# zhaotudou/HeteroFusionRCNN

Measured on AMD Instinct MI355X. Metric: KITTI frames/sec RPN train step, higher is better.
Workload: dtype f32

## Files before the change

### heterofusionrcnn_amd/csrc/xconv.hip

```cpp
#include "xconv_common.h"

namespace hf {

template <int K, bool TRANSPOSED>
__global__ __launch_bounds__(kXcThreads) void xconv_apply_kernel(long long rows, int c, const float *__restrict__ x,
                                                                const float *__restrict__ f, float *__restrict__ out)
{
    const int lane = threadIdx.x & 63;
    const long long wave = __builtin_amdgcn_readfirstlane(static_cast<int>(threadIdx.x >> 6)) +
                           static_cast<long long>(blockIdx.x) * (kXcThreads / 64);
    const long long nwaves = static_cast<long long>(gridDim.x) * (kXcThreads / 64);
    for (long long r = wave; r < rows; r += nwaves) {
        const float *xr = x + r * (K * K);
        float coef[K][K];
#pragma unroll
        for (int i = 0; i < K; ++i)
#pragma unroll
            for (int j = 0; j < K; ++j) coef[i][j] = TRANSPOSED ? xr[j * K + i] : xr[i * K + j];
        const float *fr = f + r * K * c;
        float *orow = out + r * K * c;
        for (int ch = lane; ch < c; ch += 64) {
            float v[K];
#pragma unroll
            for (int j = 0; j < K; ++j) v[j] = fr[static_cast<size_t>(j) * c + ch];
// ... 296 lines not shown
                                                                    const float *__restrict__ grad_out, float *__restrict__ grad_f,
                                                                    float *__restrict__ grad_gathered, float *__restrict__ grad_wd,
                                                                    float *__restrict__ wd_partial)
{
    const int lane = threadIdx.x & 63, wave = __builtin_amdgcn_readfirstlane(static_cast<int>(threadIdx.x >> 6));
    const int ch = blockIdx.y * 64 + lane;
    const bool live = ch < c;
    const XcSource src = xc_source(live ? ch : blockIdx.y * 64, c, c0, f, fts, GATHER ? idx : nullptr);
    if (GATHER && src.gathered && !grad_wd && !grad_gathered) return;
    float w[K][M], gw[K][M];
#pragma unroll
    for (int k = 0; k < K; ++k)
#pragma unroll
        for (int m = 0; m < M; ++m) { w[k][m] = live ? wd[(static_cast<size_t>(k) * c + ch) * M + m] : 0.f; gw[k][m] = 0.f; }
    const long long r0 = static_cast<long long>(blockIdx.x) * rows_per_block;
    const long long r1 = r0 + rows_per_block < rows ? r0 + rows_per_block : rows;
    for (long long r = r0 + wave; r < r1; r += kXcThreads / 64) {
        const float *xr = x + r * (K * K);
        float fv[K], g[M], gfx[K];
        const long long tbase = (GATHER && src.gathered) ? static_cast<long long>(static_cast<unsigned>(r) / static_cast<unsigned>(rows_per_cloud)) * n_src : 0;
#pragma unroll
        for (int j = 0; j < K; ++j) {
            const long long srow = (GATHER && src.gathered) ? tbase + idx[r * K + j] : r * K + j;
            fv[j] = live ? src.base[srow * src.stride] : 0.f;
        }
        load_m<M>(grad_out, static_cast<size_t>(r * c + (live ? ch : 0)) * M, g);
        if (!live) {
#pragma unroll
            for (int m = 0; m < M; ++m) g[m] = 0.f;
        }
#pragma unroll
        for (int k = 0; k < K; ++k) {
            float a = 0.f;
#pragma unroll
            for (int m = 0; m < M; ++m) a = a + g[m] * w[k][m];
            gfx[k] = a;
            float t = xr[k * K] * fv[0];
#pragma unroll
            for (int j = 1; j < K; ++j) t = t + xr[k * K + j] * fv[j];
#pragma unroll
            for (int m = 0; m < M; ++m) gw[k][m] = gw[k][m] + t * g[m];
        }
        float *gdst = (GATHER && src.gathered) ? (grad_gathered ? grad_gathered + (ch - c0) : nullptr) : (grad_f ? grad_f + ch : nullptr);
        if (live && gdst) {
#pragma unroll
            for (int j = 0; j < K; ++j) {
                float a = xr[j] * gfx[0];
#pragma unroll
                for (int k = 1; k < K; ++k) a = a + xr[k * K + j] * gfx[k];
                gdst[(r * K + j) * src.stride] = a;
            }
        }
    }
    if (grad_wd) {
        __shared__ float red[K * M][64];
        for (int wv = 0; wv < kXcThreads / 64; ++wv) {
            if (wave == wv && live) {
#pragma unroll
                for (int k = 0; k < K; ++k)
#pragma unroll
                    for (int m = 0; m < M; ++m) red[k * M + m][lane] = wv == 0 ? gw[k][m] : red[k * M + m][lane] + gw[k][m];
            }
            __syncthreads();
        }
        float *mine = wd_partial ? wd_partial + static_cast<size_t>(blockIdx.x) * K * c * M : nullptr;
        for (int i = threadIdx.x; i < K * M * 64; i += kXcThreads) {
            const int km = i >> 6, c2 = blockIdx.y * 64 + (i & 63);
            if (c2 < c) {
                const size_t e = (static_cast<size_t>(km / M) * c + c2) * M + km % M;
                if (mine) mine[e] = red[km][i & 63];
                else atomicAdd(&grad_wd[e], red[km][i & 63]);
            }
        }
    }
}

template <int K, int M, bool GATHER>
__global__ __launch_bounds__(kXcThreads) void xconv_dw_bwd_x_kernel(long long rows, int c, int c0, const float *__restrict__ f,
                                                                   const float *__restrict__ fts, const int *__restrict__ idx, int n_src,
                                                                   int rows_per_cloud, const float *__restrict__ wd,
                                                                   const float *__restrict__ grad_out, float *__restrict__ grad_x)
{
    extern __shared__ float lds[];
    constexpr int KK = K * K, STRIDE = KK + 1, QUADS = 16;
    const int lane = threadIdx.x & 63, w = threadIdx.x >> 6;
    float *mine = lds + static_cast<size_t>(w) * QUADS * STRIDE;
    const long long wave = w + static_cast<long long>(blockIdx.x) * (kXcThreads / 64);
    const long long nwaves = static_cast<long long>(gridDim.x) * (kXcThreads / 64);
    const int c1 = c - c0;
    for (long long r = wave; r < rows; r += nwaves) {
        float acc[K][K];
#pragma unroll
        for (int i = 0; i < K; ++i)
#pragma unroll
            for (int j = 0; j < K; ++j) acc[i][j] = 0.f;
        long long trow[K];
        if constexpr (GATHER) {
            const long long tbase = static_cast<long long>(static_cast<unsigned>(r) / static_cast<unsigned>(rows_per_cloud)) * n_src;
#pragma unroll
            for (int j = 0; j < K; ++j) trow[j] = tbase + idx[r * K + j];
        }
        for (int ch = lane; ch < c; ch += 64) {
            float fv[K], g[M];
            if constexpr (GATHER) {
                const bool gathered = ch >= c0;
                const float *base = gathered ? fts + (ch - c0) : f + ch;
                const long long stride = gathered ? c1 : c0;
#pragma unroll
                for (int j = 0; j < K; ++j) fv[j] = base[(gathered ? trow[j] : r * K + j) * stride];
            } else {
#pragma unroll
                for (int j = 0; j < K; ++j) fv[j] = f[(r * K + j) * c + ch];
            }
            load_m<M>(grad_out, static_cast<size_t>(r * c + ch) * M, g);
#pragma unroll
            for (int k = 0; k < K; ++k) {
                float a = 0.f;
#pragma unroll
                for (int m = 0; m < M; ++m) a = a + g[m] * wd[(static_cast<size_t>(k) * c + ch) * M + m];
#pragma unroll
                for (int j = 0; j < K; ++j) acc[k][j] = acc[k][j] + a * fv[j];
            }
        }
#pragma unroll
        for (int i = 0; i < K; ++i)
#pragma unroll
            for (int j = 0; j < K; ++j) {
                float v = acc[i][j];
                v = v + __int_as_float(__builtin_amdgcn_mov_dpp(__float_as_int(v), 0xb1, 0xf, 0xf, true));
                v = v + __int_as_float(__builtin_amdgcn_mov_dpp(__float_as_int(v), 0x4e, 0xf, 0xf, true));
                if ((lane & 3) == 0) mine[(lane >> 2) * STRIDE + i * K + j] = v;
            }
        __builtin_amdgcn_fence(__ATOMIC_SEQ_CST, "wavefront");
        __builtin_amdgcn_wave_barrier();
        for (int p = lane; p < KK; p += 64) {
            float s = 0.f;
#pragma unroll
            for (int l = 0; l < QUADS; ++l) s = s + mine[l * STRIDE + p];
            grad_x[r * KK + p] = s;
        }
        __builtin_amdgcn_fence(__ATOMIC_SEQ_CST, "wavefront");
        __builtin_amdgcn_wave_barrier();
    }
}

constexpr int kFtsRows = 2, kFtsEntries = 4;
typedef float f4 __attribute__((ext_vector_type(4)));

constexpr int xc_fts_pairs(int m) { return m == 1 ? 2 : 1; }

template <int K, int M, bool VEC>
__global__ __launch_bounds__(kXcThreads) void xconv_dw_bwd_fts_kernel(long long src_rows, int n_src, long long rows_per_cloud,
                                                                     int c, int c0, int rows_per_block,
                                                                     const float *__restrict__ x, const float *__restrict__ wd,
                                                                     const float *grad_out,
                                                                     const int *__restrict__ offsets, const int *__restrict__ entries,
                                                                     float *grad_fts)
{
    constexpr int NP = xc_fts_pairs(M), CPL = 2 * NP, T = kFtsRows, E = kFtsEntries, NF = CPL * M, CHUNK = NF % 4 == 0 ? 4 : 2;
    constexpr int KP = K <= 4 ? 4 : (K <= 8 ? 8 : 16), QPL = 64 / KP, NR = (T * E + QPL - 1) / QPL;
    const int lane = threadIdx.x & 63, wave = __builtin_amdgcn_readfirstlane(static_cast<int>(threadIdx.x >> 6));
    const int lq = lane / KP, lk = lane % KP < K ? lane % KP : K - 1;
    const int c1 = c - c0, col0 = blockIdx.y * (64 * CPL), cf0 = col0 + lane * CPL;
    unsigned cc[CPL];
    bool live[CPL];
#pragma unroll
    for (int i = 0; i < CPL; ++i) {
        live[i] = cf0 + i < c1;
        cc[i] = static_cast<unsigned>(c0 + (live[i] ? cf0 + i : (VEC ? col0 + i : c1 - 1)));
    }
    f2 w[K][NP][M];
#pragma unroll
    for (int k = 0; k < K; ++k)
#pragma unroll
        for (int p = 0; p < NP; ++p)
#pragma unroll
            for (int m = 0; m < M; ++m)
                w[k][p][m] = f2{wd[(static_cast<size_t>(k) * c + cc[2 * p]) * M + m], wd[(static_cast<size_t>(k) * c + cc[2 * p + 1]) * M + m]};
    __shared__ __attribute__((aligned(16))) float xs[kXcThreads / 64][T * E][KP];
    const long long s0 = static_cast<long long>(blockIdx.x) * rows_per_block;
    const long long s1 = s0 + rows_per_block < src_rows ? s0 + rows_per_block : src_rows;
    long long bb = s0 / n_src;
    for (long long sb = s0 + wave * T; sb < s1; sb += (kXcThreads / 64) * T) {
        int pos[T], hi[T];
        long long ebase[T];
        unsigned rbase[T];
        f2 acc[T][NP];
        bool more = false;
#pragma unroll
        for (int t = 0; t < T; ++t) {
            const long long s = sb + t < s1 ? sb + t : s1 - 1;
            while (s >= (bb + 1) * n_src) ++bb;
            const int pt = static_cast<int>(s - bb * n_src);
            const int *off = offsets + bb * (n_src + 1);
            ebase[t] = bb * rows_per_cloud * K;
            rbase[t] = static_cast<unsigned>(bb * rows_per_cloud);
            pos[t] = off[pt];
            hi[t] = sb + t < s1 ? off[pt + 1] : pos[t];
            more = more || pos[t] < hi[t];
#pragma unroll
            for (int p = 0; p < NP; ++p) acc[t][p] = f2{0.f, 0.f};
        }
        auto load_slots = [&](int ahead, unsigned (&slot)[NR]) {
#pragma unroll
            for (int i = 0; i < NR; ++i) {
                const int q = i * QPL + lq < T * E ? i * QPL + lq : T * E - 1, u = q % E + ahead;
                int e = 0;
                long long eb = 0;
#pragma unroll
                for (int t = 0; t < T; ++t)
                    if (q / E == t) { e = pos[t] + u < hi[t] ? pos[t] + u : 0; eb = ebase[t]; }
                slot[i] = static_cast<unsigned>(entries[eb + e]);
            }
        };
        unsigned slot[NR], slot_next[NR];
        if (more) load_slots(0, slot);
        while (more) {
            unsigned rr[T * E];
            float xv[NR];
#pragma unroll
            for (int i = 0; i < NR; ++i) {
                const int q = i * QPL + lq < T * E ? i * QPL + lq : T * E - 1;
                unsigned rb = 0;
#pragma unroll
                for (int t = 0; t < T; ++t)
                    if (q / E == t) rb = rbase[t];
// ... 243 lines not shown
                                 as_stream(stream));
}

#define HF_XDW_DISPATCH(CALL)                                                                                          \
    if (k == 8 && m == 1) { CALL(8, 1) } else if (k == 8 && m == 2) { CALL(8, 2) } else if (k == 8 && m == 3) { CALL(8, 3) }      \
    else if (k == 8 && m == 4) { CALL(8, 4) }                                                                          \
    else if (k == 4 && m == 1) { CALL(4, 1) } else if (k == 4 && m == 4) { CALL(4, 4) }    \
    else if (k == 12 && m == 1) { CALL(12, 1) } else if (k == 12 && m == 2) { CALL(12, 2) }                             \
    else return HF_EINVAL;

static void xdw_grid(long long rows, int c, dim3 &grid, int &rows_per_block, int blocks_per_cu = 8, int chunk = 64)
{
    const int cchunks = div_up(c, chunk);
    long long rchunks = (blocks_per_cu * kNumCU + cchunks - 1) / cchunks;
    if (rchunks > (rows + 3) / 4) rchunks = (rows + 3) / 4;
    if (rchunks < 1) rchunks = 1;
    rows_per_block = static_cast<int>((rows + rchunks - 1) / rchunks);
    grid = dim3(static_cast<unsigned>((rows + rows_per_block - 1) / rows_per_block), cchunks);
}

bool hf::xdw_offsets_fit(long long rows, int k, int c, long long src_rows)
{
    return rows * k * static_cast<long long>(c) < (1ll << 32) && src_rows * static_cast<long long>(c) < (1ll << 32);
}

bool hf::xdw_v2(int c, std::initializer_list<const void *> ptrs)
{
    if (c & 1) return false;
    for (const void *p : ptrs)
        if (reinterpret_cast<uintptr_t>(p) & 7) return false;
    return true;
}

void hf::xdw_pair_grid(long long rows, int c, dim3 &grid, int &rpb, int blocks_per_cu) { xdw_grid(rows, c, grid, rpb, blocks_per_cu, 128); }

static int xdw_forward(long long rows, int k, int c, int c0, int m, const float *x, const float *f, const float *fts, const int *idx,
                       int n_src, int rows_per_cloud, const float *wd, float *out, hipStream_t st)
{
    if (!xdw_offsets_fit(rows, k, c, idx ? static_cast<long long>(rows / rows_per_cloud) * n_src : 0)) return HF_EINVAL;
    dim3 grid;
    int rpb;
    xdw_pair_grid(rows, c, grid, rpb, 8);
    const bool v2 = xdw_v2(c, {f, fts, out});
#define HF_XDW_FWD_V(KK, MM, V)                                                                                        \
    if (idx) hipLaunchKernelGGL((xconv_dw_fwd_kernel<KK, MM, true, V>), grid, dim3(kXcThreads), 0, st, rows, c, c0, rpb, x, f, fts, idx, n_src, rows_per_cloud, wd, out); \
    else hipLaunchKernelGGL((xconv_dw_fwd_kernel<KK, MM, false, V>), grid, dim3(kXcThreads), 0, st, rows, c, c0, rpb, x, f, fts, idx, n_src, rows_per_cloud, wd, out);
#define HF_XDW_FWD(KK, MM) if (v2) { HF_XDW_FWD_V(KK, MM, true) } else { HF_XDW_FWD_V(KK, MM, false) }
    HF_XDW_DISPATCH(HF_XDW_FWD)
#undef HF_XDW_FWD
#undef HF_XDW_FWD_V
    return launch_status();
}

void hf::xdw_bwd_grid(long long rows, int c, dim3 &grid, int &rpb)
{
    xdw_grid(rows, c, grid, rpb, 4);
    if (rpb < 32 && rows > 32) { rpb = 32; grid.x = static_cast<unsigned>((rows + rpb - 1) / rpb); }
}

static int xdw_backward(long long rows, int k, int c, int c0, int m, const float *x, const float *f, const float *fts, const int *idx,
                        int n_src, int rows_per_cloud, const float *wd, const float *grad_out, float *grad_x, float *grad_f, float *grad_gathered,
                        float *grad_wd, hipStream_t st, float *wd_partial = nullptr)
{
    if (grad_wd && (!wd_partial || rows == 0)) {
        const int rc = hip_status(hipMemsetAsync(grad_wd, 0, sizeof(float) * static_cast<size_t>(k) * c * m, st));
        if (rc != HF_OK) return rc;
    }
    if (rows == 0) return HF_OK;
    if (!grad_wd) wd_partial = nullptr;
    if (grad_f || grad_wd || grad_gathered) {
        dim3 grid;
        int rpb;
        xdw_bwd_grid(rows, c, grid, rpb);
#define HF_XDW_BFW(KK, MM)                                                                                             \
        if (idx) hipLaunchKernelGGL((xconv_dw_bwd_fw_kernel<KK, MM, true>), grid, dim3(kXcThreads), 0, st, rows, c, c0, rpb, x, f, fts, idx, n_src, rows_per_cloud, wd, grad_out, grad_f, grad_gathered, grad_wd, wd_partial); \
        else hipLaunchKernelGGL((xconv_dw_bwd_fw_kernel<KK, MM, false>), grid, dim3(kXcThreads), 0, st, rows, c, c0, rpb, x, f, fts, idx, n_src, rows_per_cloud, wd, grad_out, grad_f, grad_gathered, grad_wd, wd_partial);
        HF_XDW_DISPATCH(HF_XDW_BFW)
#undef HF_XDW_BFW
        if (wd_partial) launch_partial_reduce(k * c * m, static_cast<int>(grid.x), wd_partial, grad_wd, st);
        const int rc = launch_status();
        if (rc != HF_OK) return rc;
    }
    if (grad_x) {
        const size_t lds = sizeof(float) * (kXcThreads / 64) * 16 * (static_cast<size_t>(k) * k + 1);
#define HF_XDW_BX(KK, MM)                                                                                              \
        if (idx) hipLaunchKernelGGL((xconv_dw_bwd_x_kernel<KK, MM, true>), dim3(grid_for(rows, kXcThreads / 64)), dim3(kXcThreads), lds, st, rows, c, c0, f, fts, idx, n_src, rows_per_cloud, wd, grad_out, grad_x); \
        else hipLaunchKernelGGL((xconv_dw_bwd_x_kernel<KK, MM, false>), dim3(grid_for(rows, kXcThreads / 64)), dim3(kXcThreads), lds, st, rows, c, c0, f, fts, idx, n_src, rows_per_cloud, wd, grad_out, grad_x);
        HF_XDW_DISPATCH(HF_XDW_BX)
#undef HF_XDW_BX
        return launch_status();
    }
    return HF_OK;
}

HF_API int hf_xconv_depthwise(long long rows, int k, int c, int m, const float *x, const float *f, const float *wd, float *out,
                              hf_stream_t stream)
{
    if (rows < 0 || c <= 0 || !x || !f || !wd || !out) return HF_EINVAL;
    if (rows == 0) return HF_OK;
    return xdw_forward(rows, k, c, c, m, x, f, nullptr, nullptr, 0, 1, wd, out, as_stream(stream));
}

HF_API int hf_xconv_depthwise_grad(long long rows, int k, int c, int m, const float *x, const float *f, const float *wd,
                                   const float *grad_out, float *grad_x, float *grad_f, float *grad_wd, hf_stream_t stream)
{
    if (rows < 0 || c <= 0 || !x || !f || !wd || !grad_out || (!grad_x && !grad_f && !grad_wd)) return HF_EINVAL;
    return xdw_backward(rows, k, c, c, m, x, f, nullptr, nullptr, 0, 1, wd, grad_out, grad_x, grad_f, nullptr, grad_wd, as_stream(stream));
}

HF_API int hf_xconv_depthwise_gather(int b, int n_src, int rows_per_cloud, int k, int c0, int c1, int m, const float *x,
                                     const float *f_delta, const float *fts, const int *idx, const float *wd, float *out,
                                     hf_stream_t stream)
{
    if (b < 0 || n_src <= 0 || rows_per_cloud < 0 || c0 <= 0 || c0 % 64 != 0 || c1 <= 0) return HF_EINVAL;
    const long long rows = static_cast<long long>(b) * rows_per_cloud;
    if (rows == 0) return HF_OK;
    if (rows > 0x7fffffffll || !x || !f_delta || !fts || !idx || !wd || !out) return HF_EINVAL;
    return xdw_forward(rows, k, c0 + c1, c0, m, x, f_delta, fts, idx, n_src, rows_per_cloud, wd, out, as_stream(stream));
}

bool hf::xdw_fts_direct(long long rows, int n_src, int rows_per_cloud, int k, int c1, int m)
{
    if (static_cast<long long>(rows_per_cloud) * k >= 8ll * n_src) return true;
    const long long staged = rows * k * c1 * static_cast<long long>(sizeof(float));
    return staged <= (8ll << 20) || (m <= 2 && staged >= (80ll << 20));
}

int hf::xdw_table_grad(long long src_rows, int n_src, int rows_per_cloud, int k, int c, int c0, int m, const float *x, const float *wd,
                          const float *grad_out, const int *offsets, const int *entries, float *grad_fts, hipStream_t st)
{
    const int c1 = c - c0, cpl = 2 * xc_fts_pairs(m);
    dim3 grid;
    int rpb;
    xdw_grid(src_rows, c1, grid, rpb, 8, 64 * cpl);
    const bool vec = c1 % cpl == 0 && ((reinterpret_cast<uintptr_t>(grad_out) | reinterpret_cast<uintptr_t>(grad_fts)) & 15) == 0;
#define HF_XDW_FTS_V(KK, MM, V) hipLaunchKernelGGL((xconv_dw_bwd_fts_kernel<KK, MM, V>), grid, dim3(kXcThreads), 0, st, src_rows, n_src, static_cast<long long>(rows_per_cloud), c, c0, rpb, x, wd, grad_out, offsets, entries, grad_fts);
#define HF_XDW_FTS(KK, MM) if (vec) { HF_XDW_FTS_V(KK, MM, true) } else { HF_XDW_FTS_V(KK, MM, false) }
    HF_XDW_DISPATCH(HF_XDW_FTS)
#undef HF_XDW_FTS
#undef HF_XDW_FTS_V
    return launch_status();
}

size_t hf::xdw_gathered_bytes(int b, int rows_per_cloud, int k, int c1)
{
    return (sizeof(float) * static_cast<size_t>(b) * rows_per_cloud * k * c1 + 255) & ~static_cast<size_t>(255);
}

HF_API size_t hf_xconv_depthwise_gather_grad_workspace(int b, int rows_per_cloud, int k, int c0, int c1, int m)
{
    if (b <= 0 || rows_per_cloud <= 0 || k <= 0 || c0 <= 0 || c1 <= 0 || m <= 0) return 0;
    dim3 grid;
    int rpb;
    xdw_bwd_grid(static_cast<long long>(b) * rows_per_cloud, c0 + c1, grid, rpb);
    return xdw_gathered_bytes(b, rows_per_cloud, k, c1) + sizeof(float) * static_cast<size_t>(grid.x) * k * (c0 + c1) * m;
}

HF_API int hf_xconv_depthwise_gather_grad(int b, int n_src, int rows_per_cloud, int k, int c0, int c1, int m, const float *x,
                                          const float *f_delta, const float *fts, const int *idx, const float *wd,
                                          const float *grad_out, const int *offsets, const int *entries, float *grad_x,
                                          float *grad_f_delta, float *grad_fts, float *grad_wd, void *workspace,
                                          size_t workspace_bytes, hf_stream_t stream)
{
    if (b < 0 || n_src <= 0 || rows_per_cloud < 0 || c0 <= 0 || c0 % 64 != 0 || c1 <= 0 || !x || !f_delta || !fts || !idx || !wd ||
        !grad_out || static_cast<long long>(b) * rows_per_cloud > 0x7fffffffll ||
        (!grad_x && !grad_f_delta && !grad_fts && !grad_wd))
        return HF_EINVAL;
// ... 24 lines not shown
```

### heterofusionrcnn_amd/csrc/xconv_bn.hip

```cpp
#include "xconv_common.h"

namespace hf {

template <int K, int M, bool V2>
__global__ __launch_bounds__(kXcThreads) void xconv_bn_fwd_kernel(long long rows, int c, int c0, int rows_per_block,
                                                                 const float *__restrict__ x, const float *__restrict__ z1,
                                                                 const float *__restrict__ gamma, const float *__restrict__ beta,
                                                                 const float *__restrict__ mean, const float *__restrict__ invstd,
                                                                 const float *__restrict__ fts, const int *__restrict__ idx, int n_src,
                                                                 int rows_per_cloud, const float *__restrict__ wd, float *__restrict__ out)
{
    const int lane = threadIdx.x & 63, wave = __builtin_amdgcn_readfirstlane(static_cast<int>(threadIdx.x >> 6));
    const int ch = blockIdx.y * 128 + 2 * lane;
    const XcPair src = xc_pair(ch, c, c0, z1, fts, true);
    const int cw = src.live ? ch : (c - 1) & ~1;
    f2 w[K][M];
#pragma unroll
    for (int k = 0; k < K; ++k)
#pragma unroll
        for (int m = 0; m < M; ++m) w[k][m] = f2{wd[(static_cast<size_t>(k) * c + cw) * M + m], wd[(static_cast<size_t>(k) * c + cw + src.hi) * M + m]};
    const int cb = src.gathered ? 0 : cw;
    const bool some_lifted = static_cast<int>(blockIdx.y) * 128 < c0;
    const f2 ba = f2{gamma[cb] * invstd[cb], gamma[cb + 1] * invstd[cb + 1]};
    const f2 bmu = f2{mean[cb], mean[cb + 1]}, bb = f2{beta[cb], beta[cb + 1]};
// ... 106 lines not shown
        }
        float *gdst = src.gathered ? (grad_gathered ? grad_gathered + (ch - c0) : nullptr) : (grad_f ? grad_f + ch : nullptr);
        if (live && gdst) {
            float ga[K];
#pragma unroll
            for (int j = 0; j < K; ++j) {
                float a = xr[j] * gfx[0];
#pragma unroll
                for (int k = 1; k < K; ++k) a = a + xr[k * K + j] * gfx[k];
                gdst[(r * K + j) * src.stride] = a;
                ga[j] = a;
            }
            if (lifted) {
#pragma unroll
                for (int j = 0; j < K; ++j) { s1 += ga[j]; s2 += ga[j] * ((xv[j] - bmu) * bis); }
            }
        }
    }
    __shared__ float red[K * M][64];
    if (lifted && grad_f) {
        for (int wv = 0; wv < kXcThreads / 64; ++wv) {
            if (wave == wv) {
                red[0][lane] = wv == 0 ? s1 : red[0][lane] + s1;
                red[1][lane] = wv == 0 ? s2 : red[1][lane] + s2;
            }
            __syncthreads();
        }
        if (wave == 0) {
            float *mine = bn_partial + static_cast<size_t>(blockIdx.x) * 2 * c0;
            mine[ch] = red[0][lane];
            mine[c0 + ch] = red[1][lane];
        }
    }
    if (grad_wd) {
        for (int wv = 0; wv < kXcThreads / 64; ++wv) {
            if (wave == wv && live) {
#pragma unroll
                for (int k = 0; k < K; ++k)
#pragma unroll
                    for (int m = 0; m < M; ++m) red[k * M + m][lane] = wv == 0 ? gw[k][m] : red[k * M + m][lane] + gw[k][m];
            }
            __syncthreads();
        }
        float *mine = wd_partial + static_cast<size_t>(blockIdx.x) * K * c * M;
        for (int i = threadIdx.x; i < K * M * 64; i += kXcThreads) {
            const int km = i >> 6, c2 = blockIdx.y * 64 + (i & 63);
            if (c2 < c) mine[(static_cast<size_t>(km / M) * c + c2) * M + km % M] = red[km][i & 63];
        }
    }
}

__global__ __launch_bounds__(kXcThreads) void xconv_bn_finalize_kernel(int c0, int nblk, const float *__restrict__ bn_partial,
                                                                      float *__restrict__ dgamma, float *__restrict__ dbeta)
{
    __shared__ double cross[2][kXcThreads / 64];
    const int ch = blockIdx.x, lane = threadIdx.x & 63, wave = threadIdx.x >> 6;
    double a = 0.0, b = 0.0;
    for (int i = threadIdx.x; i < nblk; i += kXcThreads) {
        a += static_cast<double>(bn_partial[static_cast<size_t>(i) * 2 * c0 + ch]);
        b += static_cast<double>(bn_partial[static_cast<size_t>(i) * 2 * c0 + c0 + ch]);
    }
#pragma unroll
    for (int off = 32; off > 0; off >>= 1) { a += __shfl_xor(a, off); b += __shfl_xor(b, off); }
    if (lane == 0) { cross[0][wave] = a; cross[1][wave] = b; }
    __syncthreads();
    if (threadIdx.x == 0) {
        a = cross[0][0]; b = cross[1][0];
#pragma unroll
        for (int w = 1; w < kXcThreads / 64; ++w) { a += cross[0][w]; b += cross[1][w]; }
        dbeta[ch] = static_cast<float>(a);
        dgamma[ch] = static_cast<float>(b);
    }
}

template <int K, int M>
__global__ __launch_bounds__(kXcThreads) void xconv_bn_bwd_x_kernel(long long rows, int c, int c0, const float *__restrict__ z1,
                                                                   const float *__restrict__ gamma, const float *__restrict__ beta,
                                                                   const float *__restrict__ mean, const float *__restrict__ invstd,
                                                                   const float *__restrict__ fts, const int *__restrict__ idx, int n_src,
                                                                   int rows_per_cloud, const float *__restrict__ wd,
                                                                   const float *__restrict__ grad_out, float *__restrict__ grad_x)
{
    extern __shared__ float lds[];
    constexpr int KK = K * K, STRIDE = KK + 1, QUADS = 16;
    const int lane = threadIdx.x & 63, w = threadIdx.x >> 6;
    float *mine = lds + static_cast<size_t>(w) * QUADS * STRIDE;
    const long long wave = w + static_cast<long long>(blockIdx.x) * (kXcThreads / 64);
    const long long nwaves = static_cast<long long>(gridDim.x) * (kXcThreads / 64);
    const int c1 = c - c0;
    for (long long r = wave; r < rows; r += nwaves) {
        float acc[K][K];
#pragma unroll
        for (int i = 0; i < K; ++i)
#pragma unroll
            for (int j = 0; j < K; ++j) acc[i][j] = 0.f;
        long long trow[K];
        const long long tbase = static_cast<long long>(static_cast<unsigned>(r) / static_cast<unsigned>(rows_per_cloud)) * n_src;
#pragma unroll
        for (int j = 0; j < K; ++j) trow[j] = tbase + idx[r * K + j];
        for (int ch = lane; ch < c; ch += 64) {
            float fv[K], g[M];
            const bool gathered = ch >= c0;
            const float *base = gathered ? fts + (ch - c0) : z1 + ch;
            const long long stride = gathered ? c1 : c0;
#pragma unroll
            for (int j = 0; j < K; ++j) fv[j] = base[(gathered ? trow[j] : r * K + j) * stride];
            if (ch - lane < c0) {
                const float ba = gamma[ch] * invstd[ch], bmu = mean[ch], bb = beta[ch];
#pragma unroll
                for (int j = 0; j < K; ++j) fv[j] = ba * (elu_stream(fv[j]) - bmu) + bb;
            }
            load_m<M>(grad_out, static_cast<size_t>(r * c + ch) * M, g);
#pragma unroll
            for (int k = 0; k < K; ++k) {
                float a = 0.f;
#pragma unroll
                for (int m = 0; m < M; ++m) a = a + g[m] * wd[(static_cast<size_t>(k) * c + ch) * M + m];
#pragma unroll
                for (int j = 0; j < K; ++j) acc[k][j] = acc[k][j] + a * fv[j];
            }
        }
#pragma unroll
        for (int i = 0; i < K; ++i)
#pragma unroll
            for (int j = 0; j < K; ++j) {
                float v = acc[i][j];
                v = v + __int_as_float(__builtin_amdgcn_mov_dpp(__float_as_int(v), 0xb1, 0xf, 0xf, true));
                v = v + __int_as_float(__builtin_amdgcn_mov_dpp(__float_as_int(v), 0x4e, 0xf, 0xf, true));
                if ((lane & 3) == 0) mine[(lane >> 2) * STRIDE + i * K + j] = v;
            }
        __builtin_amdgcn_fence(__ATOMIC_SEQ_CST, "wavefront");
        __builtin_amdgcn_wave_barrier();
        for (int p = lane; p < KK; p += 64) {
            float s = 0.f;
#pragma unroll
            for (int l = 0; l < QUADS; ++l) s = s + mine[l * STRIDE + p];
            grad_x[r * KK + p] = s;
        }
        __builtin_amdgcn_fence(__ATOMIC_SEQ_CST, "wavefront");
        __builtin_amdgcn_wave_barrier();
    }
}

}

using namespace hf;

#define HF_XBN_DISPATCH(CALL)                                                                                          \
    if (k == 8 && m == 1) { CALL(8, 1) } else if (k == 8 && m == 2) { CALL(8, 2) } else if (k == 8 && m == 4) { CALL(8, 4) }      \
    else return HF_EINVAL;

static bool xbn_km_ok(int k, int m) { return k == 8 && (m == 1 || m == 2 || m == 4); }

static bool xbn_shape_ok(int b, int n_src, int rows_per_cloud, int k, int c0, int c1, int m)
{
    if (b < 0 || n_src <= 0 || rows_per_cloud < 0 || c0 <= 0 || c0 % 64 != 0 || c1 <= 0 || !xbn_km_ok(k, m)) return false;
    const long long rows = static_cast<long long>(b) * rows_per_cloud;
    return rows <= 0x7fffffffll && xdw_offsets_fit(rows, k, c0 + c1, static_cast<long long>(b) * n_src);
}

static size_t xbn_align(size_t bytes) { return (bytes + 255) & ~static_cast<size_t>(255); }

HF_API int hf_xconv_depthwise_gather_bn(int b, int n_src, int rows_per_cloud, int k, int c0, int c1, int m, const float *x,
                                        const float *z1, const float *gamma, const float *beta, const float *mean,
                                        const float *invstd, const float *fts, const int *idx, const float *wd, float *out,
                                        hf_stream_t stream)
{
    if (!xbn_shape_ok(b, n_src, rows_per_cloud, k, c0, c1, m)) return HF_EINVAL;
    const long long rows = static_cast<long long>(b) * rows_per_cloud;
    if (rows == 0) return HF_OK;
    if (!x || !z1 || !gamma || !beta || !mean || !invstd || !fts || !idx || !wd || !out) return HF_EINVAL;
    const int c = c0 + c1;
    dim3 grid;
    int rpb;
    xdw_pair_grid(rows, c, grid, rpb, 8);
    const bool v2 = xdw_v2(c, {z1, fts, out});
    hipStream_t st = as_stream(stream);
#define HF_XBN_FWD_V(KK, MM, V)                                                                                        \
    hipLaunchKernelGGL((xconv_bn_fwd_kernel<KK, MM, V>), grid, dim3(kXcThreads), 0, st, rows, c, c0, rpb, x, z1, gamma, beta, mean, invstd, fts, idx, n_src, rows_per_cloud, wd, out);
#define HF_XBN_FWD(KK, MM) if (v2) { HF_XBN_FWD_V(KK, MM, true) } else { HF_XBN_FWD_V(KK, MM, false) }
    HF_XBN_DISPATCH(HF_XBN_FWD)
#undef HF_XBN_FWD
#undef HF_XBN_FWD_V
    return launch_status();
}

static size_t xbn_base_bytes(int b, int rows_per_cloud, int k, int c0, int c1, int m)
{
    return xbn_align(hf_xconv_depthwise_gather_grad_workspace(b, rows_per_cloud, k, c0, c1, m));
}

HF_API size_t hf_xconv_depthwise_gather_bn_grad_workspace(int b, int rows_per_cloud, int k, int c0, int c1, int m)
{
    if (b <= 0 || rows_per_cloud <= 0 || k <= 0 || c0 <= 0 || c1 <= 0 || m <= 0) return 0;
    dim3 grid;
    int rpb;
    xdw_bwd_grid(static_cast<long long>(b) * rows_per_cloud, c0 + c1, grid, rpb);
    return xbn_base_bytes(b, rows_per_cloud, k, c0, c1, m) + sizeof(float) * static_cast<size_t>(grid.x) * 2 * c0;
}

HF_API int hf_xconv_depthwise_gather_bn_grad(int b, int n_src, int rows_per_cloud, int k, int c0, int c1, int m, const float *x,
                                             const float *z1, const float *gamma, const float *beta, const float *mean,
                                             const float *invstd, const float *fts, const int *idx, const float *wd,
                                             const float *grad_out, const int *offsets, const int *entries, float *grad_x,
                                             float *grad_f, float *grad_fts, float *grad_wd, float *dgamma, float *dbeta,
                                             void *workspace, size_t workspace_bytes, hf_stream_t stream)
{
    if (!xbn_shape_ok(b, n_src, rows_per_cloud, k, c0, c1, m) || !x || !z1 || !gamma || !beta || !mean || !invstd || !fts || !idx || !wd ||
        !grad_out || (!grad_x && !grad_f && !grad_fts && !grad_wd))
        return HF_EINVAL;
    if ((grad_fts && (!offsets || !entries)) || (grad_f && (!dgamma || !dbeta))) return HF_EINVAL;
    hipStream_t st = as_stream(stream);
    const long long rows = static_cast<long long>(b) * rows_per_cloud, src_rows = static_cast<long long>(b) * n_src;
    const int c = c0 + c1;
    if (rows == 0) {
        int rc = HF_OK;
        if (grad_wd) rc = hip_status(hipMemsetAsync(grad_wd, 0, sizeof(float) * static_cast<size_t>(k) * c * m, st));
        if (rc == HF_OK && grad_fts && src_rows > 0) rc = hip_status(hipMemsetAsync(grad_fts, 0, sizeof(float) * static_cast<size_t>(src_rows) * c1, st));
        if (rc == HF_OK && grad_f) rc = hip_status(hipMemsetAsync(dgamma, 0, sizeof(float) * c0, st));
        if (rc == HF_OK && grad_f) rc = hip_status(hipMemsetAsync(dbeta, 0, sizeof(float) * c0, st));
        return rc;
    }
    if (!workspace || workspace_bytes < hf_xconv_depthwise_gather_bn_grad_workspace(b, rows_per_cloud, k, c0, c1, m)) return HF_EWORKSPACE;
    const bool want_fts = grad_fts != nullptr;
    const bool direct = want_fts && xdw_fts_direct(rows, n_src, rows_per_cloud, k, c1, m);
    unsigned char *ws = static_cast<unsigned char *>(workspace);
    float *gathered = (want_fts && !direct) ? static_cast<float *>(workspace) : nullptr;
    float *wd_partial = grad_wd ? reinterpret_cast<float *>(ws + xdw_gathered_bytes(b, rows_per_cloud, k, c1)) : nullptr;
    float *bn_partial = reinterpret_cast<float *>(ws + xbn_base_bytes(b, rows_per_cloud, k, c0, c1, m));
    if (grad_f || grad_wd || gathered) {
        dim3 grid;
        int rpb;
        xdw_bwd_grid(rows, c, grid, rpb);
#define HF_XBN_BFW(KK, MM)                                                                                             \
        hipLaunchKernelGGL((xconv_bn_bwd_fw_kernel<KK, MM>), grid, dim3(kXcThreads), 0, st, rows, c, c0, rpb, x, z1, gamma, beta, mean, invstd, fts, idx, n_src, rows_per_cloud, wd, grad_out, grad_f, gathered, grad_wd, wd_partial, bn_partial);
        HF_XBN_DISPATCH(HF_XBN_BFW)
#undef HF_XBN_BFW
        if (grad_wd) launch_partial_reduce(k * c * m, static_cast<int>(grid.x), wd_partial, grad_wd, st);
        if (grad_f) hipLaunchKernelGGL(xconv_bn_finalize_kernel, dim3(c0), dim3(kXcThreads), 0, st, c0, static_cast<int>(grid.x), bn_partial, dgamma, dbeta);
        const int rc = launch_status();
        if (rc != HF_OK) return rc;
    }
    if (grad_x) {
        const size_t lds = sizeof(float) * (kXcThreads / 64) * 16 * (static_cast<size_t>(k) * k + 1);
#define HF_XBN_BX(KK, MM)                                                                                              \
        hipLaunchKernelGGL((xconv_bn_bwd_x_kernel<KK, MM>), dim3(grid_for(rows, kXcThreads / 64)), dim3(kXcThreads), lds, st, rows, c, c0, z1, gamma, beta, mean, invstd, fts, idx, n_src, rows_per_cloud, wd, grad_out, grad_x);
        HF_XBN_DISPATCH(HF_XBN_BX)
#undef HF_XBN_BX
        const int rc = launch_status();
        if (rc != HF_OK) return rc;
    }
    if (gathered) return hf_group_point_grad_gather(b, n_src, c1, rows_per_cloud, k, c1, 0, gathered, offsets, entries, grad_fts, stream);
    if (direct) return xdw_table_grad(src_rows, n_src, rows_per_cloud, k, c, c0, m, x, wd, grad_out, offsets, entries, grad_fts, st);
    return HF_OK;
}
```

### heterofusionrcnn_amd/csrc/xconv_common.h

```cpp
#pragma once
#include "hf_common.h"

#include <initializer_list>

namespace hf {

template <int M>
__device__ __forceinline__ void store_m(float *base, size_t elem, const float (&v)[M])
{
    float *p = base + elem;
    if constexpr (M == 4 || M == 8) {
        if ((reinterpret_cast<uintptr_t>(base) & 15) == 0) {
#pragma unroll
            for (int q = 0; q < M / 4; ++q) reinterpret_cast<float4 *>(p)[q] = make_float4(v[4 * q], v[4 * q + 1], v[4 * q + 2], v[4 * q + 3]);
            return;
        }
    } else if constexpr (M == 2) {
        if ((reinterpret_cast<uintptr_t>(base) & 7) == 0) { *reinterpret_cast<float2 *>(p) = make_float2(v[0], v[1]); return; }
    }
#pragma unroll
    for (int m = 0; m < M; ++m) p[m] = v[m];
}
template <int M>
__device__ __forceinline__ void load_m(const float *base, size_t elem, float (&v)[M])
// ... 63 lines not shown
        }
    }
}

constexpr int kXcRows = 2;

struct XcCloud {
    long long next;
    unsigned tbase;
};

__device__ __forceinline__ unsigned xc_tbase(XcCloud &cl, long long r, int rows_per_cloud, int n_src)
{
    while (r >= cl.next) { cl.next += rows_per_cloud; cl.tbase += static_cast<unsigned>(n_src); }
    return cl.tbase;
}

__device__ __forceinline__ XcCloud xc_cloud(long long r, int rows_per_cloud, int n_src)
{
    const long long b = r / rows_per_cloud;
    return XcCloud{(b + 1) * rows_per_cloud, static_cast<unsigned>(b * n_src)};
}

template <int K, bool GATHER, bool V2>
__device__ __forceinline__ void xc_gather_row(const XcPair &s, long long r, unsigned tbase, const int *__restrict__ idx,
                                              unsigned lstride, unsigned c1, f2 (&fv)[K])
{
    const unsigned rk = static_cast<unsigned>(r) * K;
#pragma unroll
    for (int j = 0; j < K; ++j) {
        const unsigned lo = (rk + j) * lstride;
        unsigned off = lo;
        if constexpr (GATHER) {
            const unsigned go = (tbase + static_cast<unsigned>(idx[rk + j])) * c1;
            off = s.gathered ? go : lo;
        }
        fv[j] = ld_pair<V2>(s.base + off, s.hi);
    }
}

template <int K>
struct XcXRows {
    static constexpr int KK = K * K, Q = (KK + 63) / 64;
    float v[kXcRows][Q];
    __device__ __forceinline__ void load(const float *__restrict__ x, const long long (&rr)[kXcRows], int lane)
    {
#pragma unroll
        for (int i = 0; i < kXcRows; ++i)
#pragma unroll
            for (int q = 0; q < Q; ++q) {
                const int p = lane + 64 * q;
                v[i][q] = x[rr[i] * KK + (p < KK ? p : KK - 1)];
            }
    }
    __device__ __forceinline__ void stage(float (*xs)[KK], int lane) const
    {
        __builtin_amdgcn_fence(__ATOMIC_SEQ_CST, "wavefront");
        __builtin_amdgcn_wave_barrier();
#pragma unroll
        for (int i = 0; i < kXcRows; ++i)
#pragma unroll
            for (int q = 0; q < Q; ++q)
                if (lane + 64 * q < KK) xs[i][lane + 64 * q] = v[i][q];
        __builtin_amdgcn_fence(__ATOMIC_SEQ_CST, "wavefront");
        __builtin_amdgcn_wave_barrier();
    }
};

struct XcSource {
    const float *base;
    long long stride;
    bool gathered;
};

__device__ __forceinline__ XcSource xc_source(int ch, int c, int c0, const float *f, const float *fts, const int *idx)
{
    XcSource s;
    if (idx == nullptr) { s.base = f + ch; s.stride = c; s.gathered = false; }
    else if (ch - (ch & 63) < c0) { s.base = f + ch; s.stride = c0; s.gathered = false; }
    else { s.base = fts + (ch - c0); s.stride = c - c0; s.gathered = true; }
    return s;
}

void xdw_pair_grid(long long rows, int c, dim3 &grid, int &rpb, int blocks_per_cu);
void xdw_bwd_grid(long long rows, int c, dim3 &grid, int &rpb);
bool xdw_offsets_fit(long long rows, int k, int c, long long src_rows);
bool xdw_v2(int c, std::initializer_list<const void *> ptrs);
bool xdw_fts_direct(long long rows, int n_src, int rows_per_cloud, int k, int c1, int m);
size_t xdw_gathered_bytes(int b, int rows_per_cloud, int k, int c1);
int xdw_table_grad(long long src_rows, int n_src, int rows_per_cloud, int k, int c, int c0, int m, const float *x, const float *wd,
                   const float *grad_out, const int *offsets, const int *entries, float *grad_fts, hipStream_t st);

}
```

Baseline: 325.9.

## Rewrite xconv grad_x backward with LDS-cached weights, prefetch, and cross-lane fold

Replaces the two duplicated grad_x backward kernels with one shared body. When the weights fit (at most 64 channel-trip × K·M slots), it stages the depthwise weights and the BN affine parameters in LDS once per block. The body software-pipelines the next channel trip's feature and gradient loads, uses packed f2 multiply-adds, and reduces the K×K accumulators with permlane/DPP lane folds instead of per-wave LDS scratch with barriers. It also caches the per-cloud index base and vectorises the grad_out loads. The cost is extra register pressure from the double-buffered trips and the 64-wide accumulator flattening, plus a block-wide LDS fill before any work starts.

```diff
diff --git a/heterofusionrcnn_amd/csrc/xconv.hip b/heterofusionrcnn_amd/csrc/xconv.hip
--- a/heterofusionrcnn_amd/csrc/xconv.hip
+++ b/heterofusionrcnn_amd/csrc/xconv.hip
@@ -402,66 +402,8 @@
                                                                    const float *__restrict__ grad_out, float *__restrict__ grad_x)
 {
     extern __shared__ float lds[];
-    constexpr int KK = K * K, STRIDE = KK + 1, QUADS = 16;
-    const int lane = threadIdx.x & 63, w = threadIdx.x >> 6;
-    float *mine = lds + static_cast<size_t>(w) * QUADS * STRIDE;
-    const long long wave = w + static_cast<long long>(blockIdx.x) * (kXcThreads / 64);
-    const long long nwaves = static_cast<long long>(gridDim.x) * (kXcThreads / 64);
-    const int c1 = c - c0;
-    for (long long r = wave; r < rows; r += nwaves) {
-        float acc[K][K];
-#pragma unroll
-        for (int i = 0; i < K; ++i)
-#pragma unroll
-            for (int j = 0; j < K; ++j) acc[i][j] = 0.f;
-        long long trow[K];
-        if constexpr (GATHER) {
-            const long long tbase = static_cast<long long>(static_cast<unsigned>(r) / static_cast<unsigned>(rows_per_cloud)) * n_src;
-#pragma unroll
-            for (int j = 0; j < K; ++j) trow[j] = tbase + idx[r * K + j];
-        }
-        for (int ch = lane; ch < c; ch += 64) {
-            float fv[K], g[M];
-            if constexpr (GATHER) {
-                const bool gathered = ch >= c0;
-                const float *base = gathered ? fts + (ch - c0) : f + ch;
-                const long long stride = gathered ? c1 : c0;
-#pragma unroll
-                for (int j = 0; j < K; ++j) fv[j] = base[(gathered ? trow[j] : r * K + j) * stride];
-            } else {
-#pragma unroll
-                for (int j = 0; j < K; ++j) fv[j] = f[(r * K + j) * c + ch];
-            }
-            load_m<M>(grad_out, static_cast<size_t>(r * c + ch) * M, g);
-#pragma unroll
-            for (int k = 0; k < K; ++k) {
-                float a = 0.f;
-#pragma unroll
-                for (int m = 0; m < M; ++m) a = a + g[m] * wd[(static_cast<size_t>(k) * c + ch) * M + m];
-#pragma unroll
-                for (int j = 0; j < K; ++j) acc[k][j] = acc[k][j] + a * fv[j];
-            }
-        }
-#pragma unroll
-        for (int i = 0; i < K; ++i)
-#pragma unroll
-            for (int j = 0; j < K; ++j) {
-                float v = acc[i][j];
-                v = v + __int_as_float(__builtin_amdgcn_mov_dpp(__float_as_int(v), 0xb1, 0xf, 0xf, true));
-                v = v + __int_as_float(__builtin_amdgcn_mov_dpp(__float_as_int(v), 0x4e, 0xf, 0xf, true));
-                if ((lane & 3) == 0) mine[(lane >> 2) * STRIDE + i * K + j] = v;
-            }
-        __builtin_amdgcn_fence(__ATOMIC_SEQ_CST, "wavefront");
-        __builtin_amdgcn_wave_barrier();
-        for (int p = lane; p < KK; p += 64) {
-            float s = 0.f;
-#pragma unroll
-            for (int l = 0; l < QUADS; ++l) s = s + mine[l * STRIDE + p];
-            grad_x[r * KK + p] = s;
-        }
-        __builtin_amdgcn_fence(__ATOMIC_SEQ_CST, "wavefront");
-        __builtin_amdgcn_wave_barrier();
-    }
+    xc_bwd_x_body<K, M, GATHER, false>(rows, c, c0, f, nullptr, nullptr, nullptr, nullptr, fts, idx, n_src, rows_per_cloud, wd, grad_out,
+                                       grad_x, lds);
 }
 
 constexpr int kFtsRows = 2, kFtsEntries = 4;
@@ -871,7 +813,7 @@
         if (rc != HF_OK) return rc;
     }
     if (grad_x) {
-        const size_t lds = sizeof(float) * (kXcThreads / 64) * 16 * (static_cast<size_t>(k) * k + 1);
+        const size_t lds = xc_bwd_x_lds_bytes(c, 0, k * m);
 #define HF_XDW_BX(KK, MM)                                                                                              \
         if (idx) hipLaunchKernelGGL((xconv_dw_bwd_x_kernel<KK, MM, true>), dim3(grid_for(rows, kXcThreads / 64)), dim3(kXcThreads), lds, st, rows, c, c0, f, fts, idx, n_src, rows_per_cloud, wd, grad_out, grad_x); \
         else hipLaunchKernelGGL((xconv_dw_bwd_x_kernel<KK, MM, false>), dim3(grid_for(rows, kXcThreads / 64)), dim3(kXcThreads), lds, st, rows, c, c0, f, fts, idx, n_src, rows_per_cloud, wd, grad_out, grad_x);
diff --git a/heterofusionrcnn_amd/csrc/xconv_bn.hip b/heterofusionrcnn_amd/csrc/xconv_bn.hip
--- a/heterofusionrcnn_amd/csrc/xconv_bn.hip
+++ b/heterofusionrcnn_amd/csrc/xconv_bn.hip
@@ -212,64 +212,7 @@
                                                                    const float *__restrict__ grad_out, float *__restrict__ grad_x)
 {
     extern __shared__ float lds[];
-    constexpr int KK = K * K, STRIDE = KK + 1, QUADS = 16;
-    const int lane = threadIdx.x & 63, w = threadIdx.x >> 6;
-    float *mine = lds + static_cast<size_t>(w) * QUADS * STRIDE;
-    const long long wave = w + static_cast<long long>(blockIdx.x) * (kXcThreads / 64);
-    const long long nwaves = static_cast<long long>(gridDim.x) * (kXcThreads / 64);
-    const int c1 = c - c0;
-    for (long long r = wave; r < rows; r += nwaves) {
-        float acc[K][K];
-#pragma unroll
-        for (int i = 0; i < K; ++i)
-#pragma unroll
-            for (int j = 0; j < K; ++j) acc[i][j] = 0.f;
-        long long trow[K];
-        const long long tbase = static_cast<long long>(static_cast<unsigned>(r) / static_cast<unsigned>(rows_per_cloud)) * n_src;
-#pragma unroll
-        for (int j = 0; j < K; ++j) trow[j] = tbase + idx[r * K + j];
-        for (int ch = lane; ch < c; ch += 64) {
-            float fv[K], g[M];
-            const bool gathered = ch >= c0;
-            const float *base = gathered ? fts + (ch - c0) : z1 + ch;
-            const long long stride = gathered ? c1 : c0;
-#pragma unroll
-            for (int j = 0; j < K; ++j) fv[j] = base[(gathered ? trow[j] : r * K + j) * stride];
-            if (ch - lane < c0) {
-                const float ba = gamma[ch] * invstd[ch], bmu = mean[ch], bb = beta[ch];
-#pragma unroll
-                for (int j = 0; j < K; ++j) fv[j] = ba * (elu_stream(fv[j]) - bmu) + bb;
-            }
-            load_m<M>(grad_out, static_cast<size_t>(r * c + ch) * M, g);
-#pragma unroll
-            for (int k = 0; k < K; ++k) {
-                float a = 0.f;
-#pragma unroll
-                for (int m = 0; m < M; ++m) a = a + g[m] * wd[(static_cast<size_t>(k) * c + ch) * M + m];
-#pragma unroll
-                for (int j = 0; j < K; ++j) acc[k][j] = acc[k][j] + a * fv[j];
-            }
-        }
-#pragma unroll
-        for (int i = 0; i < K; ++i)
-#pragma unroll
-            for (int j = 0; j < K; ++j) {
-                float v = acc[i][j];
-                v = v + __int_as_float(__builtin_amdgcn_mov_dpp(__float_as_int(v), 0xb1, 0xf, 0xf, true));
-                v = v + __int_as_float(__builtin_amdgcn_mov_dpp(__float_as_int(v), 0x4e, 0xf, 0xf, true));
-                if ((lane & 3) == 0) mine[(lane >> 2) * STRIDE + i * K + j] = v;
-            }
-        __builtin_amdgcn_fence(__ATOMIC_SEQ_CST, "wavefront");
-        __builtin_amdgcn_wave_barrier();
-        for (int p = lane; p < KK; p += 64) {
-            float s = 0.f;
-#pragma unroll
-            for (int l = 0; l < QUADS; ++l) s = s + mine[l * STRIDE + p];
-            grad_x[r * KK + p] = s;
-        }
-        __builtin_amdgcn_fence(__ATOMIC_SEQ_CST, "wavefront");
-        __builtin_amdgcn_wave_barrier();
-    }
+    xc_bwd_x_body<K, M, true, true>(rows, c, c0, z1, gamma, beta, mean, invstd, fts, idx, n_src, rows_per_cloud, wd, grad_out, grad_x, lds);
 }
 
 }
@@ -372,7 +315,7 @@
         if (rc != HF_OK) return rc;
     }
     if (grad_x) {
-        const size_t lds = sizeof(float) * (kXcThreads / 64) * 16 * (static_cast<size_t>(k) * k + 1);
+        const size_t lds = xc_bwd_x_lds_bytes(c, c0, k * m);
 #define HF_XBN_BX(KK, MM)                                                                                              \
         hipLaunchKernelGGL((xconv_bn_bwd_x_kernel<KK, MM>), dim3(grid_for(rows, kXcThreads / 64)), dim3(kXcThreads), lds, st, rows, c, c0, z1, gamma, beta, mean, invstd, fts, idx, n_src, rows_per_cloud, wd, grad_out, grad_x);
         HF_XBN_DISPATCH(HF_XBN_BX)
diff --git a/heterofusionrcnn_amd/csrc/xconv_common.h b/heterofusionrcnn_amd/csrc/xconv_common.h
--- a/heterofusionrcnn_amd/csrc/xconv_common.h
+++ b/heterofusionrcnn_amd/csrc/xconv_common.h
@@ -169,6 +169,279 @@
     return s;
 }
 
+
+template <int M>
+__device__ __forceinline__ void xc_load_m(const float *arg, const float *p, float (&v)[M])
+{
+    if constexpr (M == 4) {
+        if ((reinterpret_cast<uintptr_t>(arg) & 15) == 0) {
+            const float4 t = *reinterpret_cast<const float4 *>(p);
+            v[0] = t.x; v[1] = t.y; v[2] = t.z; v[3] = t.w;
+            return;
+        }
+    } else if constexpr (M == 2) {
+        if ((reinterpret_cast<uintptr_t>(arg) & 7) == 0) { const float2 t = *reinterpret_cast<const float2 *>(p); v[0] = t.x; v[1] = t.y; return; }
+    }
+#pragma unroll
+    for (int m = 0; m < M; ++m) v[m] = p[m];
+}
+
+struct XcCloudDiv {
+    long long first, next;
+    long long tbase;
+};
+
+__device__ __forceinline__ long long xc_tbase_div(XcCloudDiv &cl, long long r, int rows_per_cloud, int n_src)
+{
+    if (r >= cl.next || r < cl.first) {
+        const long long b = static_cast<long long>(static_cast<unsigned>(r) / static_cast<unsigned>(rows_per_cloud));
+        cl.first = b * rows_per_cloud;
+        cl.next = cl.first + rows_per_cloud;
+        cl.tbase = b * n_src;
+    }
+    return cl.tbase;
+}
+
+template <int CTRL>
+__device__ __forceinline__ float xc_dpp(float v)
+{
+    return __int_as_float(__builtin_amdgcn_update_dpp(0, __float_as_int(v), CTRL, 0xf, 0xf, true));
+}
+
+template <int KK, int OFF, int N>
+__device__ __forceinline__ void xc_lane_fold(float (&v)[KK], int lane)
+{
+    static_assert(N == 64 || N == 16, "chunks of 64 or 16 entries");
+    typedef unsigned u2 __attribute__((ext_vector_type(2)));
+#pragma unroll
+    for (int i = 0; i < N / 2; ++i) {
+        const u2 s = __builtin_amdgcn_permlane32_swap(__float_as_uint(v[OFF + i]), __float_as_uint(v[OFF + i + N / 2]), false, false);
+        v[OFF + i] = __uint_as_float(s.x) + __uint_as_float(s.y);
+    }
+#pragma unroll
+    for (int i = 0; i < N / 4; ++i) {
+        const u2 s = __builtin_amdgcn_permlane16_swap(__float_as_uint(v[OFF + i]), __float_as_uint(v[OFF + i + N / 4]), false, false);
+        v[OFF + i] = __uint_as_float(s.x) + __uint_as_float(s.y);
+    }
+    const bool b3 = (lane & 8) != 0, b2 = (lane & 4) != 0;
+#pragma unroll
+    for (int i = 0; i < N / 8; ++i) {
+        const float lo = v[OFF + i], hi = v[OFF + i + N / 8];
+        v[OFF + i] = (b3 ? hi : lo) + xc_dpp<0x128>(b3 ? lo : hi);
+    }
+#pragma unroll
+    for (int i = 0; i < N / 16; ++i) {
+        const float lo = v[OFF + i], hi = v[OFF + i + N / 16];
+        v[OFF + i] = (b2 ? hi : lo) + xc_dpp<0x141>(b2 ? lo : hi);
+    }
+    if constexpr (N == 64) {
+        const bool b1 = (lane & 2) != 0, b0 = (lane & 1) != 0;
+#pragma unroll
+        for (int i = 0; i < 2; ++i) {
+            const float lo = v[OFF + i], hi = v[OFF + i + 2];
+            v[OFF + i] = (b1 ? hi : lo) + xc_dpp<0x4e>(b1 ? lo : hi);
+        }
+        const float lo = v[OFF], hi = v[OFF + 1];
+        v[OFF] = (b0 ? hi : lo) + xc_dpp<0xb1>(b0 ? lo : hi);
+    } else {
+        v[OFF] = v[OFF] + xc_dpp<0x4e>(v[OFF]);
+        v[OFF] = v[OFF] + xc_dpp<0xb1>(v[OFF]);
+    }
+}
+
+template <int KK, int OFF = 0>
+__device__ __forceinline__ void xc_store_dx(float (&acc)[KK], int lane, float *__restrict__ dst)
+{
+    static_assert((KK - OFF) % 64 == 0 || (KK - OFF) % 64 == 16, "K * K is a multiple of 64, or 16 more");
+    if constexpr (KK - OFF >= 64) {
+        xc_lane_fold<KK, OFF, 64>(acc, lane);
+        dst[OFF + lane] = acc[OFF];
+        xc_store_dx<KK, OFF + 64>(acc, lane, dst);
+    } else if constexpr (KK - OFF == 16) {
+        xc_lane_fold<KK, OFF, 16>(acc, lane);
+        if ((lane & 3) == 0) dst[OFF + (lane >> 2)] = acc[OFF];
+    }
+}
+
+__device__ __forceinline__ const float *xc_at(const float *base, unsigned byte_off)
+{
+    return reinterpret_cast<const float *>(reinterpret_cast<const char *>(base) + byte_off);
+}
+
+constexpr int kXcWdSlots = 64;
+inline __host__ __device__ bool xc_bwd_x_fast(int c, int km) { return ((c + 63) >> 6) * km <= kXcWdSlots; }
+inline size_t xc_bwd_x_lds_bytes(int c, int c0_bn, int km)
+{
+    return xc_bwd_x_fast(c, km) ? sizeof(float) * (64 * static_cast<size_t>((c + 63) >> 6) * km + 3 * static_cast<size_t>(c0_bn)) : 0;
+}
+
+template <int K, int M>
+struct XcTrip {
+    float fv[K], g[M];
+};
+
+template <int K, int M, bool GATHER, bool BN, bool FAST>
+__device__ __forceinline__ void xc_bwd_x_rows(long long rows, int c, int c0, const float *__restrict__ f,
+                                              const float *__restrict__ gamma, const float *__restrict__ beta,
+                                              const float *__restrict__ mean, const float *__restrict__ invstd,
+                                              const float *__restrict__ fts, const int *__restrict__ idx, int n_src, int rows_per_cloud,
+                                              const float *__restrict__ wd, const float *__restrict__ grad_out,
+                                              float *__restrict__ grad_x, float *lds)
+{
+    constexpr int KK = K * K, KM = K * M;
+    const int lane = threadIdx.x & 63, w = __builtin_amdgcn_readfirstlane(static_cast<int>(threadIdx.x >> 6));
+    const long long wave = w + static_cast<long long>(blockIdx.x) * (kXcThreads / 64);
+    const long long nwaves = static_cast<long long>(gridDim.x) * (kXcThreads / 64);
+    const int trips = (c + 63) >> 6, c1 = c - c0;
+    const unsigned lstride = GATHER ? c0 : c;
+    float *bnl = lds + trips * KM * 64;
+    if constexpr (FAST) {
+        for (int i = threadIdx.x; i < trips * KM * 64; i += kXcThreads) {
+            const int l = i & 63, s = i >> 6, t = s / KM, km = s - t * KM, ch = 64 * t + l;
+            lds[i] = ch < c ? wd[(static_cast<size_t>(km / M) * c + ch) * M + km % M] : 0.f;
+        }
+        if constexpr (BN) {
+            for (int i = threadIdx.x; i < c0; i += kXcThreads) {
+                bnl[i] = gamma[i] * invstd[i];
+                bnl[c0 + i] = mean[i];
+                bnl[2 * c0 + i] = beta[i];
+            }
+        }
+        __syncthreads();
+    }
+    if (wave >= rows) return;
+
+    int nidx[K];
+    auto load_idx = [&](long long r) {
+        if constexpr (GATHER) {
+            const long long rc = r < rows ? r : rows - 1;
+#pragma unroll
+            for (int j = 0; j < K; ++j) nidx[j] = idx[rc * K + j];
+        }
+    };
+    XcCloudDiv cl{0, 0, 0};
+    const float *fl = f, *go = grad_out, *tj[K];
+    auto set_row = [&](long long r) {
+        fl = f + r * K * static_cast<long long>(lstride);
+        go = grad_out + r * c * static_cast<long long>(M);
+        if constexpr (GATHER) {
+            const long long tb = xc_tbase_div(cl, r, rows_per_cloud, n_src);
+#pragma unroll
+            for (int j = 0; j < K; ++j) tj[j] = fts + static_cast<unsigned long long>(tb + nidx[j]) * static_cast<unsigned>(c1);
+        }
+    };
+    auto load_trip = [&](int t, XcTrip<K, M> &o) {
+        const int ch = 64 * t + lane;
+        const unsigned cc = ch < c ? ch : c - 1;
+        const float *bj[K];
+        unsigned sub = 0;
+        if (GATHER && 64 * t >= c0) {
+            sub = c0;
+#pragma unroll
+            for (int j = 0; j < K; ++j) bj[j] = tj[j];
+        } else {
+#pragma unroll
+            for (int j = 0; j < K; ++j) bj[j] = fl + j * static_cast<size_t>(lstride);
+        }
+        const unsigned off = (cc - sub) * 4u;
+#pragma unroll
+        for (int j = 0; j < K; ++j) o.fv[j] = *xc_at(bj[j], off);
+        xc_load_m<M>(grad_out, xc_at(go, cc * (4u * M)), o.g);
+    };
+
+    long long r = wave;
+    int t = 0;
+    load_idx(r);
+    set_row(r);
+    XcTrip<K, M> cur, nxt;
+    load_trip(0, cur);
+    static_assert(K % 2 == 0, "pairs of j");
+    f2 acc[K][K / 2];
+    for (;;) {
+        const bool last = t + 1 == trips;
+        const long long rn = last ? r + nwaves : r;
+        const int tn = last ? 0 : t + 1;
+        const bool more = rn < rows;
+        if (t == 0) load_idx(r + nwaves);
+        if (last) set_row(more ? rn : r);
+        load_trip(tn, nxt);
+        const int ch = 64 * t + lane;
+        const bool live = ch < c;
+        const unsigned cc = live ? ch : c - 1;
+        if (BN && 64 * t < c0) {
+            float ba, bmu, bb;
+            if constexpr (FAST) { ba = bnl[cc]; bmu = bnl[c0 + cc]; bb = bnl[2 * c0 + cc]; }
+            else { ba = gamma[cc] * invstd[cc]; bmu = mean[cc]; bb = beta[cc]; }
+#pragma unroll
+            for (int j = 0; j < K; ++j) cur.fv[j] = ba * (elu_stream(cur.fv[j]) - bmu) + bb;
+        }
+        f2 ap[K / 2];
+        {
+            const float *wt = lds + (t * KM * 64 + lane);
+            auto wv = [&](int k, int m) { return FAST ? wt[(k * M + m) * 64] : wd[(static_cast<size_t>(k) * c + cc) * M + m]; };
+#pragma unroll
+            for (int i = 0; i < K / 2; ++i) {
+                ap[i] = cur.g[0] * f2{wv(2 * i, 0), wv(2 * i + 1, 0)};
+#pragma unroll
+                for (int m = 1; m < M; ++m) ap[i] = ap[i] + cur.g[m] * f2{wv(2 * i, m), wv(2 * i + 1, m)};
+            }
+        }
+        f2 fp[K / 2];
+#pragma unroll
+        for (int i = 0; i < K / 2; ++i) fp[i] = f2{cur.fv[2 * i], cur.fv[2 * i + 1]};
+        if (t == 0) {
+            if (live) {
+#pragma unroll
+                for (int k = 0; k < K; ++k)
+#pragma unroll
+                    for (int i = 0; i < K / 2; ++i) acc[k][i] = ap[k / 2][k % 2] * fp[i];
+            } else {
+#pragma unroll
+                for (int k = 0; k < K; ++k)
+#pragma unroll
+                    for (int i = 0; i < K / 2; ++i) acc[k][i] = f2{0.f, 0.f};
+            }
+        } else if (live) {
+#pragma unroll
+            for (int k = 0; k < K; ++k) {
+                f2 p[K / 2];
+#pragma unroll
+                for (int i = 0; i < K / 2; ++i) p[i] = ap[k / 2][k % 2] * fp[i];
+                __builtin_amdgcn_sched_barrier(0);
+#pragma unroll
+                for (int i = 0; i < K / 2; ++i) acc[k][i] = acc[k][i] + p[i];
+                __builtin_amdgcn_sched_barrier(0);
+            }
+        }
+        if (last) {
+            float flat[KK];
+#pragma unroll
+            for (int k = 0; k < K; ++k)
+#pragma unroll
+                for (int i = 0; i < K / 2; ++i) { flat[k * K + 2 * i] = acc[k][i].x; flat[k * K + 2 * i + 1] = acc[k][i].y; }
+            xc_store_dx<KK>(flat, lane, grad_x + r * KK);
+        }
+        if (!more) break;
+        cur = nxt;
+        r = rn;
+        t = tn;
+    }
+}
+
+template <int K, int M, bool GATHER, bool BN>
+__device__ __forceinline__ void xc_bwd_x_body(long long rows, int c, int c0, const float *__restrict__ f,
+                                              const float *__restrict__ gamma, const float *__restrict__ beta,
+                                              const float *__restrict__ mean, const float *__restrict__ invstd,
+                                              const float *__restrict__ fts, const int *__restrict__ idx, int n_src, int rows_per_cloud,
+                                              const float *__restrict__ wd, const float *__restrict__ grad_out,
+                                              float *__restrict__ grad_x, float *lds)
+{
+    if (xc_bwd_x_fast(c, K * M))
+        xc_bwd_x_rows<K, M, GATHER, BN, true>(rows, c, c0, f, gamma, beta, mean, invstd, fts, idx, n_src, rows_per_cloud, wd, grad_out, grad_x, lds);
+    else
+        xc_bwd_x_rows<K, M, GATHER, BN, false>(rows, c, c0, f, gamma, beta, mean, invstd, fts, idx, n_src, rows_per_cloud, wd, grad_out, grad_x, lds);
+}
+
 void xdw_pair_grid(long long rows, int c, dim3 &grid, int &rpb, int blocks_per_cu);
 void xdw_bwd_grid(long long rows, int c, dim3 &grid, int &rpb);
 bool xdw_offsets_fit(long long rows, int k, int c, long long src_rows);
```

New measurement: 330.0 (median of 6 runs). +1.3%, better.
